# barlettacarmen/CrCNN

Hardware: AMD Instinct MI355X
Metric: encrypted images/sec (higher is better)
Workload: dtype u64

## Files before the change

crcnn_amd/binding.py:

```python
import ctypes
import os
import re

import numpy as np

_HERE = os.path.dirname(os.path.abspath(__file__))
LIB_PATH = os.path.join(_HERE, "lib", "libcrcnn_hip.so")
HEADER = os.path.join(os.path.dirname(_HERE), "include", "crcnn_hip.h")

u64 = ctypes.c_uint64
PU = ctypes.POINTER(u64)
VP = ctypes.c_void_p
CI = ctypes.c_int
SZ = ctypes.c_size_t

COEFF, NTT, NTTP, NTTL, NTTL1, NTTLC, NTTLS = 0, 1, 2, 3, 4, 5, 6


class CrcError(RuntimeError):
    def __init__(self, status, what=""):
        self.status = status
        super().__init__(f"{what}: {_strerror(status)} (status {status}, hip error {_lib.crc_last_hip_error() if _lib else '?'})")


# ... 47 lines not shown
    L.crc_event_create.argtypes = [VP, ctypes.POINTER(VP)]; L.crc_event_destroy.argtypes = [VP, VP]; L.crc_event_record.argtypes = [VP, VP, VP]
    L.crc_event_elapsed_ms.argtypes = [VP, VP, VP, ctypes.POINTER(ctypes.c_float)]
    L.crc_stream_create.argtypes = [VP, ctypes.POINTER(VP)]; L.crc_stream_destroy.argtypes = [VP, VP]; L.crc_stream_wait_event.argtypes = [VP, VP, VP]
    L.crc_host_alloc.argtypes = [VP, SZ, ctypes.POINTER(VP)]; L.crc_host_free.argtypes = [VP, VP]
    L.crc_host_thread_limit.argtypes = []
    L.crc_encode_f32.argtypes = [VP, ctypes.POINTER(ctypes.c_float), SZ, PU, ctypes.POINTER(ctypes.c_int32)]
    L.crc_encode_f64.argtypes = [VP, ctypes.POINTER(ctypes.c_double), SZ, PU, ctypes.POINTER(ctypes.c_int32)]
    L.crc_decode.restype = ctypes.c_double; L.crc_decode.argtypes = [VP, PU]
    L.crc_bn_invstd_f32.argtypes = [ctypes.POINTER(ctypes.c_float), SZ, ctypes.POINTER(ctypes.c_float)]
    L.crc_plain_to_ntt.argtypes = [VP, VP, SZ, VP, VP]
    L.crc_encode_f32_compact.argtypes = [VP, ctypes.POINTER(ctypes.c_float), SZ, PU, ctypes.POINTER(ctypes.c_int32)]
    L.crc_plain_expand.argtypes = [VP, VP, SZ, VP, VP]
    L.crc_plain_to_delta.argtypes = [VP, VP, SZ, CI, VP, VP]
    L.crc_ntt_fwd.argtypes = [VP, VP, SZ, CI, VP]
    L.crc_ntt_inv.argtypes = [VP, VP, SZ, CI, VP]
    L.crc_ntt_fwd_bsk.argtypes = [VP, VP, SZ, VP]
    L.crc_ntt_inv_bsk.argtypes = [VP, VP, SZ, VP]
    L.crc_add.argtypes = [VP, VP, VP, SZ, CI, VP]
    L.crc_add_plain.argtypes = [VP, VP, VP, SZ, SZ, CI, VP]
    L.crc_multiply_plain_ntt.argtypes = [VP, VP, VP, SZ, SZ, CI, VP]
    L.crc_multiply_plain.argtypes = [VP, VP, VP, SZ, SZ, VP]
    L.crc_conv2d_work_bytes.restype = SZ; L.crc_conv2d_work_bytes.argtypes = [VP] + [CI] * 10
    L.crc_conv2d.argtypes = [VP, VP, VP, VP] + [CI] * 11 + [VP, VP, VP]
    L.crc_conv2d_fold_pool.argtypes = [VP, VP, VP, VP] + [CI] * 8 + [VP, VP, VP]
    L.crc_conv2d_hoist_pool.argtypes = [VP, VP, VP, VP] + [CI] * 6 + [VP, VP, VP]
    L.crc_dense_work_bytes.restype = SZ; L.crc_dense_work_bytes.argtypes = [VP, CI, CI, CI, CI]
    L.crc_dense.argtypes = [VP, VP, VP, VP, CI, CI, CI, CI, CI, VP, VP, VP]
    L.crc_pool.argtypes = [VP, VP] + [CI] * 8 + [VP, CI, VP, VP]
    L.crc_batchnorm.argtypes = [VP, VP, CI, CI, CI, CI, VP, VP, CI, VP]
    L.crc_pad.argtypes = [VP, VP] + [CI] * 9 + [VP, VP]
# ... 601 lines not shown
        if isinstance(x, DBuf):
            return x.ptr
        if hasattr(x, "data_ptr"):
            return x.data_ptr()
        return int(x)

    def plain_to_ntt(self, d_plain, count, d_out):
        _chk(self.L.crc_plain_to_ntt(self.c, self.p(d_plain), count, self.p(d_out), self.stream), "crc_plain_to_ntt")

    def plain_to_delta(self, d_plain, count, form, d_out):
        _chk(self.L.crc_plain_to_delta(self.c, self.p(d_plain), count, form, self.p(d_out), self.stream), "crc_plain_to_delta")

    def ntt_fwd(self, d_ct, count, size=2):
        _chk(self.L.crc_ntt_fwd(self.c, self.p(d_ct), count, size, self.stream), "crc_ntt_fwd")

    def ntt_inv(self, d_ct, count, size=2):
        _chk(self.L.crc_ntt_inv(self.c, self.p(d_ct), count, size, self.stream), "crc_ntt_inv")

    def add(self, d_acc, d_b, count, size=2):
        _chk(self.L.crc_add(self.c, self.p(d_acc), self.p(d_b), count, size, self.stream), "crc_add")

    def add_plain(self, d_ct, d_delta, count, group, sign=1):
        _chk(self.L.crc_add_plain(self.c, self.p(d_ct), self.p(d_delta), count, group, sign, self.stream), "crc_add_plain")

    def multiply_plain_ntt(self, d_ct, d_w, count, group, size=2):
        _chk(self.L.crc_multiply_plain_ntt(self.c, self.p(d_ct), self.p(d_w), count, group, size, self.stream), "crc_multiply_plain_ntt")

    def multiply_plain(self, d_ct, d_w, count, group):
        _chk(self.L.crc_multiply_plain(self.c, self.p(d_ct), self.p(d_w), count, group, self.stream), "crc_multiply_plain")

# ... 539 lines not shown
```

crcnn_amd/csrc/abi.hip:

```cpp
#include <cstdlib>
#include <cstring>
#include <vector>
#include "kernels.h"
#include "chacha.h"
#include "work_arena.h"

#define CHECK_CTX(c) do { if (!(c) || (c)->device < 0) return CRC_ERR_INVALID_ARGUMENT; \
        int dev_ = -1; if (hipGetDevice(&dev_) != hipSuccess || dev_ != (c)->device) HIPCHK(hipSetDevice((c)->device)); } while (0)
#define RUN(x) do { int rc_ = (x); if (rc_) return rc_; } while (0)
static inline hipStream_t S(void *s) { return (hipStream_t)s; }
static inline bool form_ok(int f) { return f == CRC_COEFF || f == CRC_NTT; }
static inline bool nform_ok(int f) { return f == CRC_COEFF || f == CRC_NTT || f == CRC_NTTP; }
static inline bool lform_ok(int f) { return nform_ok(f) || f == CRC_NTTL; }
static inline bool limb_in(int f) { return f == CRC_NTTL || f == CRC_NTTLS; }
static inline u64 *work_base(void *d_work) { return WorkArena(d_work).take<u64>(0); }
static inline size_t work_bytes(size_t words) { WorkArena a; a.take<u64>(words); return a.bytes(); }

extern "C" int crc_plain_to_ntt(crc_ctx *c, const uint64_t *d_plain, size_t count, uint64_t *d_out, void *stream)
{
    CHECK_CTX(c); if (!d_plain || !d_out) return CRC_ERR_INVALID_ARGUMENT;
    return k_plain_ntt(c, d_plain, count, 1, true, d_out, S(stream));
}
extern "C" int crc_plain_expand(crc_ctx *c, const uint64_t *d_compact, size_t count, uint64_t *d_plain, void *stream)
{
    CHECK_CTX(c); if (!d_compact || !d_plain) return CRC_ERR_INVALID_ARGUMENT;
    return k_plain_expand(c, d_compact, count, d_plain, S(stream));
}
extern "C" int crc_plain_to_delta(crc_ctx *c, const uint64_t *d_plain, size_t count, int form, uint64_t *d_out, void *stream)
{
    CHECK_CTX(c); if (!d_plain || !d_out || !form_ok(form)) return CRC_ERR_INVALID_ARGUMENT;
    return k_plain_ntt(c, d_plain, count, 2, form == CRC_NTT, d_out, S(stream));
}

extern "C" int crc_ntt_fwd(crc_ctx *c, uint64_t *d_ct, size_t count, int size, void *stream)
{
    CHECK_CTX(c); if (!d_ct || size < 1) return CRC_ERR_INVALID_ARGUMENT;
    return k_ntt_ct(c, false, d_ct, d_ct, count, size, false, S(stream), nullptr, 0, 0);
}
extern "C" int crc_ntt_inv(crc_ctx *c, uint64_t *d_ct, size_t count, int size, void *stream)
{
    CHECK_CTX(c); if (!d_ct || size < 1) return CRC_ERR_INVALID_ARGUMENT;
    return k_ntt_ct(c, true, d_ct, d_ct, count, size, false, S(stream), nullptr, 0, 0);
}
extern "C" int crc_ntt_fwd_bsk(crc_ctx *c, uint64_t *d_rows, size_t count, void *stream)
{
    CHECK_CTX(c); if (!d_rows) return CRC_ERR_INVALID_ARGUMENT;
    return k_ntt_ct(c, false, d_rows, d_rows, count, 1, true, S(stream), nullptr, 0, 0);
}
extern "C" int crc_ntt_inv_bsk(crc_ctx *c, uint64_t *d_rows, size_t count, void *stream)
{
    CHECK_CTX(c); if (!d_rows) return CRC_ERR_INVALID_ARGUMENT;
    return k_ntt_ct(c, true, d_rows, d_rows, count, 1, true, S(stream), nullptr, 0, 0);
}
// ... 105 lines not shown
    L.out_form = out_form == CRC_NTTLC && P == 1 ? CRC_NTTL : out_form;
    L.Bs = conv1_sub_batch(c, B, w, nf, L.out_form);
    L.Xr = a.take<signed char>(k_limb_conv1_image_bytes(c, L.Bs, w, nf));
    if (L.out_form != CRC_NTTLC) L.Ys = a.take<u64>(k_limb_result_words(c, L.Bs, nf, P));
    if (in_form == CRC_COEFF) L.buf = a.take<u64>((size_t)L.Bs * in.xd * in.yd * crc_ct_words(c, 2));
    return L;
}
static int conv2d_limb1(crc_ctx *c, const uint64_t *d_x, const void *d_wl, const uint64_t *d_bias, int B, const Window &in, int nf, int in_form, int out_form,
                        uint64_t *d_y, void *d_work, hipStream_t st, int bxf = 1, int byf = 1)
{
    const int P = in.boxed(bxf, byf).P(), in_cts = in.xd * in.yd;
    WorkArena a(d_work);
    const Limb1Work L = limb1_layout(c, B, in, bxf, byf, nf, in_form, out_form, a);
    out_form = L.out_form;
    const size_t ctw = crc_ct_words(c, 2);
    for (int b0 = 0; b0 < B; b0 += L.Bs) {
        const int Bn = B - b0 < L.Bs ? B - b0 : L.Bs;
        const u64 *xn = d_x + (size_t)b0 * in_cts * ctw; bool packed = in_form == CRC_NTTP;
        if (in_form == CRC_COEFF) { RUN(k_ntt_ct(c, false, xn, L.buf, (size_t)Bn * in_cts, 2, false, st, nullptr, 0, 0, 0, 0)); xn = L.buf; packed = false; }
        RUN(k_limb_conv1(c, xn, packed, L.Xr, (const signed char *)d_wl, L.Ys, out_form == CRC_NTTLC ? (signed char *)d_y : nullptr, B, b0,
            out_form != CRC_COEFF ? d_bias : nullptr, Bn, in, nf, st, bxf, byf));
        if (out_form == CRC_NTTLC) continue;
        if (out_form == CRC_NTTL) return k_limb_result_to_limb(c, L.Ys, (signed char *)d_y, B, nf * P, st);
        RUN(k_limb_result_to_rows(c, L.Ys, d_y + (size_t)b0 * nf * P * ctw, (size_t)Bn * nf * P * 2, out_form == CRC_NTTP, st));
    }
    if (out_form == CRC_COEFF) RUN(k_ntt_ct(c, true, d_y, d_y, (size_t)B * nf * P, 2, false, st, d_bias, 1, (size_t)P, nf));
    return CRC_OK;
}
struct LimbWork { u64 *Ys; signed char *Xl; u64 *buf; };
static LimbWork limb_layout(const crc_ctx *c, int B, const LayerShape &s, int in_form, WorkArena &a)
{
    LimbWork L{};
    L.Ys = a.take<u64>(k_limb_result_words(c, B, s.nf, s.w.P()));
    if (!limb_in(in_form)) L.Xl = a.take<signed char>(k_limb_tensor_bytes(c, B, s.zd, s.w.xd * s.w.yd));
    if (in_form == CRC_COEFF) L.buf = a.take<u64>((size_t)B * s.zd * s.w.xd * s.w.yd * crc_ct_words(c, 2));
    return L;
// ... 1427 lines not shown
```

crcnn_amd/csrc/ctx.cpp:

```cpp
#include "ctx.h"
#include "host_parallel.h"
#include <algorithm>
#include <cstring>
#include <cstdlib>
#include <string>

typedef unsigned __int128 u128;

static thread_local int g_last_hip = 0;
int crc_set_hip_error(hipError_t e) { g_last_hip = (int)e; return CRC_ERR_HIP; }

extern "C" int crc_last_hip_error(void) { return g_last_hip; }
extern "C" int crc_version(void) { return 100; }
extern "C" const char *crc_strerror(int s)
{
    switch (s) {
    case CRC_OK: return "ok";
    case CRC_ERR_INVALID_ARGUMENT: return "invalid argument";
    case CRC_ERR_PARAMETERS: return "encryption parameters are not set correctly";
    case CRC_ERR_HIP: return "HIP runtime error";
    case CRC_ERR_UNSUPPORTED: return "unsupported parameter combination";
    case CRC_ERR_IO: return "I/O error";
    case CRC_ERR_NOT_FOUND: return "not found";
    case CRC_ERR_COMM: return "RCCL error";
// ... 131 lines not shown
    auto geti = [](const char *name, long long dflt) { const char *e = getenv(name); return e && *e ? atoll(e) : dflt; };
    t.no_fold = getenv("CRC_NO_FOLD") ? 1 : 0;
    t.ntt_inv61_loose = getenv("CRC_NTT_INV61_LOOSE") ? 1 : 0;
    t.mfma_order = (int)geti("CRC_MFMA_ORDER", -1);
    t.mfma_variant = (int)geti("CRC_MFMA_VARIANT", 2);
    { const int v = (int)geti("CRC_MFMA_RING", 0); t.mfma_ring = v >= 3 && v <= 5 ? v : 0; }
    { const int v = (int)geti("CRC_CONV1_WAVES", 0); t.conv1_waves = v == 8 || v == 12 ? v : 0; }
    t.conv1_narrow = (int)geti("CRC_CONV1_NARROW", 1);
    { const int v = (int)geti("CRC_CONV1_FORM", 0); t.conv1_form = v == 1 || v == 2 ? v : 0; }
    t.hoist_pool = geti("CRC_HOIST_POOL", 1) ? 1 : 0;
    { const int v = (int)geti("CRC_HOIST_RT", 0); t.hoist_rt = v == 1 || v == 2 ? v : 0; }
    { const int v = (int)geti("CRC_BSGS_JT", 0); t.bsgs_jt = v == 1 || v == 2 ? v : 0; }
    { const int v = (int)geti("CRC_PLANES_BATCH", 0); t.planes_batch = v == 1 || v == 2 ? v : 0; }
    { const int v = (int)geti("CRC_CONV_JT", 0); t.conv_jt = v == 2 || v == 4 || v == 8 ? v : 0; }
    t.conv1_box = geti("CRC_CONV1_BOX", 1) ? 1 : 0;
    { const long long v = geti("CRC_CONV1_PASS_BYTES", 0); t.conv1_pass_bytes = v > 0 ? v : 0; }
    { const int v = (int)geti("CRC_LIMB_PACK_GROUP", 1); t.limb_pack_group = v > 0 ? v : 1; }
    t.mac2_cfg = (int)geti("CRC_MAC2_CFG", 0);
    t.mac_order = (int)geti("CRC_MAC_ORDER", -1);
    t.mac_regstage = (int)geti("CRC_MAC_REGSTAGE", 0);
    t.mac_stream = (int)geti("CRC_MAC_STREAM", 1);
    t.mac2_dbg = (int)geti("CRC_MAC2_DBG", 0);
    t.relin_path = (int)geti("CRC_RELIN_PATH", 0);
    t.sq_path = (int)geti("CRC_SQ_PATH", 0);
    t.sq_chunk = (int)geti("CRC_SQ_CHUNK", 0);
    t.sq_fuse = (int)geti("CRC_SQ_FUSE", -1);
    t.f64_radix = (int)geti("CRC_F64_RADIX", 0);
    t.f64_wave = (int)geti("CRC_F64_WAVE", -1);
    t.ntt_wave = (int)geti("CRC_NTT_WAVE", -1);
    t.mfma_min_steps = (int)geti("CRC_MFMA_MIN_STEPS", 0);
// ... 7 lines not shown
    if (!c || !name) return CRC_ERR_INVALID_ARGUMENT;
    const std::string s(name);
    CrcTuning &t = c->tune;
    if (s == "mfma_order") t.mfma_order = (int)value;
    else if (s == "mfma_variant") t.mfma_variant = (int)value;
    else if (s == "mfma_ring") t.mfma_ring = value >= 3 && value <= 5 ? (int)value : 0;
    else if (s == "conv1_waves") t.conv1_waves = value == 8 || value == 12 ? (int)value : 0;
    else if (s == "conv1_narrow") t.conv1_narrow = (int)value;
    else if (s == "conv1_form") t.conv1_form = value == 1 || value == 2 ? (int)value : 0;
    else if (s == "hoist_pool") t.hoist_pool = value ? 1 : 0;
    else if (s == "hoist_rt") t.hoist_rt = value == 1 || value == 2 ? (int)value : 0;
    else if (s == "bsgs_jt") t.bsgs_jt = value == 1 || value == 2 ? (int)value : 0;
    else if (s == "planes_batch") t.planes_batch = value == 1 || value == 2 ? (int)value : 0;
    else if (s == "conv_jt") t.conv_jt = value == 2 || value == 4 || value == 8 ? (int)value : 0;
    else if (s == "conv1_box") t.conv1_box = value ? 1 : 0;
    else if (s == "conv1_pass_bytes") t.conv1_pass_bytes = value > 0 ? value : 0;
    else if (s == "limb_pack_group") t.limb_pack_group = value > 0 ? (int)value : 1;
    else if (s == "mac2_cfg") t.mac2_cfg = (int)value;
    else if (s == "mac_order") t.mac_order = (int)value;
    else if (s == "mac_regstage") t.mac_regstage = (int)value;
    else if (s == "mac_stream") t.mac_stream = (int)value;
    else if (s == "ntt_inv61_loose") t.ntt_inv61_loose = value ? 1 : 0;
    else if (s == "relin_path") t.relin_path = (int)value;
    else if (s == "sq_path") t.sq_path = (int)value;
    else if (s == "sq_chunk") t.sq_chunk = (int)value;
    else if (s == "sq_fuse") t.sq_fuse = (int)value;
    else if (s == "f64_radix") t.f64_radix = (int)value;
    else if (s == "f64_wave") t.f64_wave = (int)value;
    else if (s == "ntt_wave") t.ntt_wave = (int)value;
    else if (s == "mfma_min_steps") t.mfma_min_steps = (int)value;
// ... 435 lines not shown
```

crcnn_amd/csrc/ctx.h:

```cpp
#pragma once
#include <hip/hip_runtime.h>
#include <atomic>
#include <mutex>
#include <unordered_map>
#include <vector>
#include "modarith.h"
#include "f64mod.h"
#include "../../include/crcnn_hip.h"

#define CRC_MAXK 8
#define CRC_MAXB (CRC_MAXK + 2)

struct PlainParams {
    u64 threshold;
    u64 inc[CRC_MAXK];
    int fast;
    u64 delta[CRC_MAXK];
    u64 uhi[CRC_MAXK];
};

struct BehzParams {
    int k, ka, kb;
    u64 t;
    u64 m_tilde, m_sk;
// ... 49 lines not shown
    ModParams m;
    u64 root, inv_n;
    std::vector<u64> rp, srp, irp2, sirp2;
    std::vector<u64> irp, sirp;
};

struct CrcTuning {
    int no_fold = 0;
    int ntt_inv61_loose = 0;
    int mfma_order = -1;
    int mfma_variant = 2;
    int mfma_ring = 0;
    int conv1_waves = 0;
    int conv1_narrow = 1;
    int conv1_box = 1;
    int hoist_rt = 0;
    int bsgs_jt = 0;
    int planes_batch = 0;
    int conv_jt = 0;
    int hoist_pool = 1;
    int conv1_form = 0;
    long long conv1_pass_bytes = 0;
    int limb_pack_group = 1;
    int mac2_cfg = 0;
    int mac_order = -1;
    int mac_regstage = 0;
    int mac_stream = 1;
    int mac2_dbg = 0;
    int ntt_split = 1;
    int relin_mac_ct = 0;
// ... 67 lines not shown
```

crcnn_amd/csrc/kernels.h:

```cpp
#pragma once
#include "ctx.h"
#include "window.h"

static inline unsigned xcd_grid(size_t groups, unsigned G) { return (unsigned)((groups + 7) / 8 * 8 * G); }

int k_ntt_ct(crc_ctx *c, bool inv, const u64 *src, u64 *dst, size_t count, int size, bool bsk, hipStream_t st,
             const u64 *addend, int add_sign, size_t add_group, int add_mod = 0, int pack_out = 0);
int k_ntt_ct_fwd_mul(crc_ctx *c, u64 *ct, size_t count, const u64 *w, size_t group, hipStream_t st);
int k_ntt_ct_fwd_fma(crc_ctx *c, u64 *ct, size_t count, const u64 *u, const u64 *key, hipStream_t st);
int k_ntt_ct_fwd_negmul(crc_ctx *c, u64 *ct, size_t count, const u64 *sk, hipStream_t st);
int k_ntt_ct_poly0(crc_ctx *c, const u64 *src, u64 *dst, size_t count, hipStream_t st);
int k_ntt_ct_addct(crc_ctx *c, const u64 *src, u64 *dst, size_t count, const u64 *addct, int add_size, hipStream_t st);
int k_ntt_ct_head_add(crc_ctx *c, const u64 *src, int src_size, u64 *dst, size_t count, const u64 *addrows, hipStream_t st);
int k_spread_ntt(crc_ctx *c, const u64 *src, size_t items, u64 *dst, hipStream_t st);
int k_digit_ntt(crc_ctx *c, const u64 *src, int src_size, int src_poly, size_t count, int D, const unsigned char *dig_i, const unsigned char *dig_shift, int dbc,
                u64 *dst, hipStream_t st, int pack_out = 0);
int k_square_intt(crc_ctx *c, const u64 *src, u64 *dst, size_t count, bool bsk, hipStream_t st, const u64 *opt_mul = nullptr, bool *applied = nullptr);
int k_multiply_intt(crc_ctx *c, const u64 *x, const u64 *y, u64 *dst, size_t count, bool bsk, hipStream_t st, const u64 *opt_mul = nullptr, bool *applied = nullptr);
int k_ntt_ct_inv_scaled(crc_ctx *c, const u64 *src, u64 *dst, size_t count, int size, const u64 *mul, const u64 *mul_s, hipStream_t st);
int k_plain_ntt(crc_ctx *c, const u64 *d_plain, size_t count, int mode, bool do_ntt, u64 *d_out, hipStream_t st);
int k_plain_expand(crc_ctx *c, const u64 *d_compact, size_t count, u64 *d_plain, hipStream_t st);
int k_rowwise(crc_ctx *c, u64 *acc, const u64 *b, size_t count, int size, int op, int sign, size_t group, size_t gmod, hipStream_t st);
int k_pool(crc_ctx *c, const u64 *x, u64 *y, int B, int zd, const Window &w, const u64 *mul, hipStream_t st, int pack_out = 0);
int k_pad(crc_ctx *c, const u64 *x, u64 *y, int B, int zd, int xd, int yd, int px0, int px1, int py0, int py1, hipStream_t st);
// ... 103 lines not shown
```

crcnn_amd/csrc/kernels.hip:

```cpp
#include "kernels.h"
#include <type_traits>
#include <cstdlib>

struct NttArgs {
    const u64 *src; u64 *dst;
    const ModParams *mods; const ulonglong2 *w;
    int n, logn;
    int mod_base, mod_count;
    int src_rows_per_item;
    size_t rows;
    int pack_out;
    int src_ct_rows, dst_ct_rows;
    int prologue;
    int D, src_size, src_poly; unsigned long long dig_mask;
    size_t pairs;
    u64 post_mul[CRC_MAXK], post_mul_s[CRC_MAXK];
    const u64 *fma_u, *fma_k;
    unsigned long long fma_group;
    int opt_mul;
    unsigned char dig_i[48], dig_shift[48];
    const u64 *addend; int add_sign; int rows_per_ct; long long add_group;
    int add_mod;
    int add_mode, add_size;
    int fma_neg;
    PlainParams pp;
};

__device__ __forceinline__ u64 plain_lift(u64 c, const PlainParams &pp, int i, const ModParams &m)
{
    if (pp.fast) return c >= pp.threshold ? c + pp.inc[i] : c;
    const u64 r = barrett128(c, 0, m);
    return c >= pp.threshold ? addmod(r, pp.inc[i], m.q) : r;
}

#include "ntt_device.h"
#include "ntt_f64.h"
__device__ __forceinline__ u64 split28v(u64 v) { return (v & 0x0fffffffULL) | ((v >> 28) << 32); }

template <bool INV, bool LAZY, int PRO>
__device__ __forceinline__ void ntt_rows_body(const NttArgs &a)
{
    extern __shared__ u64 sm[];
    const int n = a.n, logn = a.logn, tid = threadIdx.x, nt = blockDim.x;
    size_t row = blockIdx.x;
    if (INV && (PRO == 4 || PRO == 6)) {
        size_t pair; unsigned p;
        if (!xcd_group(blockIdx.x, 3, a.pairs, pair, p)) return;
        row = ((pair / a.mod_count) * 3 + p) * a.mod_count + pair % a.mod_count;
    }
    const int mloc = (int)(row % a.mod_count);
    const int mi = a.mod_base + mloc;
// ... 83 lines not shown
        for (int s = 2 * tid; s < n; s += 2 * nt) {
            ulonglong2 v = sm_load_pair64(sm, s);
            v.x = fin(v.x); v.y = fin(v.y);
            if (add) {
                const ulonglong2 ad = ld2(add + s);
                if (a.add_sign > 0) { v.x = addmod(v.x, ad.x, q); v.y = addmod(v.y, ad.y, q); } else { v.x = submod(v.x, ad.x, q); v.y = submod(v.y, ad.y, q); }
            }
            st2(dst + s, v.x, v.y);
        }
    }
}

template <bool INV, bool LAZY, int PRO>
__global__ void __launch_bounds__(1024) ntt_rows_kernel(NttArgs a) { ntt_rows_body<INV, LAZY, PRO>(a); }

template <bool INV, int PRO, int CS, bool UNS, int FMA = 0>
__global__ void __launch_bounds__(CS == 1 ? 128 : CS == 2 ? 256 : CS == 3 ? 512 : 1024, 4) ntt_rows_wave_kernel(NttArgs a)
{
    constexpr int E = 16 >> CS, C = 1 << CS;
    extern __shared__ u64 sm[];
    const int n = a.n, tid = threadIdx.x;
    size_t row = blockIdx.x;
    if (INV && (PRO == 4 || PRO == 6)) {
        size_t pair; unsigned p;
        if (!xcd_group(blockIdx.x, 3, a.pairs, pair, p)) return;
        row = ((pair / a.mod_count) * 3 + p) * a.mod_count + pair % a.mod_count;
    }
    const int mloc = (int)(row % a.mod_count), mi = a.mod_base + mloc;
    const ModParams m = a.mods[mi];
    const u64 q = m.q, q2 = m.two_q;
    const float rq = 1.0f / (float)((u32)(q >> 32) + 1);
    const ulonglong2 *W = a.w + (size_t)mi * n, *W1 = W + (n >> 1);
    u64 *dst = a.dst + row * (size_t)n;
    auto pt = [&](int c, int e) { return E * tid + e + 1024 * c; };
    if (!INV) {
        const size_t srow = a.dst_ct_rows ? (row / a.dst_ct_rows) * a.src_ct_rows + row % a.dst_ct_rows : (a.src_rows_per_item ? (row / a.mod_count) : row);
        const u64 *src = a.src + srow * (size_t)n;
        u64 x[16];
#pragma unroll
        for (int c = 0; c < C; c++) {
            if constexpr (E == 1) x[c] = src[pt(c, 0)];
            else {
#pragma unroll
                for (int e = 0; e < E; e += 2) { const ulonglong2 v = ld2(src + pt(c, e)); x[c * E + e] = v.x; x[c * E + e + 1] = v.y; }
            }
        }
#pragma unroll
        for (int e = 0; e < E; e++) {
            u64 y[C];
#pragma unroll
            for (int c = 0; c < C; c++) y[c] = x[c * E + e];
            fwd_stages<CS, true>(y, W, 1, 0, q, q2);
#pragma unroll
            for (int c = 0; c < C; c++) sm[swz<3>(pt(c, e))] = y[c];
        }
        __syncthreads();
        const bool fma_lazy = m.fold != 0 && m.bits >= 53;
        u64_local_passes_fwd<true>(sm, W, n, q, q2);
#pragma unroll 2
        for (int u = 0; u < 8; u++) {
// ... 311 lines not shown
                if (a.add_mode == 2) add = a.addend + ((ct * a.add_size + p) * a.mod_count + mloc) * (size_t)n;
                else if (p == 0) { size_t g = ct / a.add_group; if (a.add_mod) g %= a.add_mod; add = a.addend + (g * a.mod_count + mloc) * (size_t)n; }
            }
        } else if (a.addend) add = a.addend + row * (size_t)n;
        for (int s = tid; s < n; s += nt) {
            u64 v = sm[lpad(s)];
            if (LAZY) v = reduce_small(v, q, q2, rq);
            else { v = v >= q2 ? v - q2 : v; v = v >= q ? v - q : v; }
            if (add) v = (INV && a.add_sign < 0) ? submod(v, add[s], q) : addmod(v, add[s], q);
            dst[s] = (!INV && a.pack_out) ? split28v(v) : v;
        }
        __syncthreads();
    }
}

static int ntt_launch(crc_ctx *c, bool inv, NttArgs &a, size_t rows, hipStream_t st)
{
    if (rows == 0) return CRC_OK;
    a.mods = c->d_mods; a.n = c->n; a.logn = c->logn;
    a.w = reinterpret_cast<const ulonglong2 *>(inv ? c->d_irp2 : c->d_rp);
    int nt = c->n / 8; if (nt < 64) nt = 64; if (nt > 1024) nt = 1024;
    size_t lds = (size_t)c->n * 8;
    if (lds > 128 * 1024) return CRC_ERR_UNSUPPORTED;
    bool lazy = true;
    for (int i = a.mod_base; i < a.mod_base + a.mod_count; i++) if (c->tabs[i].m.bits > 57 || c->tabs[i].m.bits < 45) lazy = false;
    const int cus = c->cus;
    if ((a.prologue == 3 && inv) || ((a.prologue == 4 || a.prologue == 5 || a.prologue == 6) && !inv)) return CRC_ERR_INVALID_ARGUMENT;
    const bool two_src = a.prologue == 6;
    if (a.prologue == 4 || two_src) rows = xcd_grid(a.pairs, 3);
    {
        const int sel = c->tune.ntt_wave < 0 ? 47 : c->tune.ntt_wave;
        const int bit = c->n == 8192 ? 0 : c->n == 4096 ? 1 : c->n == 16384 ? (a.prologue ? 3 : 2) : c->n == 2048 ? 5 : -1;
        if (bit >= 0 && ((sel >> bit) & 1) && lazy && !a.addend && (a.prologue == 0 || a.prologue == 4 || a.prologue == 5 || two_src)) {
            lds = (size_t)c->n * 8;
            bool uns = inv && !(sel & 16);
            for (int i = 0; i < a.mod_count; i++) uns = uns && c->tabs[a.mod_base + i].m.q < (1ull << 55);
            if (uns) {
                a.w = reinterpret_cast<const ulonglong2 *>(c->d_irp);
                for (int i = 0; i < a.mod_count; i++) {
                    const HostNtt &T = c->tabs[a.mod_base + i]; const u64 q = T.m.q;
                    const u64 pm = a.prologue == 5 || a.opt_mul ? (u64)(((unsigned __int128)a.post_mul[i] * T.inv_n) % q) : T.inv_n;
                    a.post_mul[i] = pm; a.post_mul_s[i] = (u64)(((unsigned __int128)pm << 64) / q);
                }
                if (a.opt_mul) a.opt_mul = 2;
            }
            const int cs = c->logn - 10;
#define WAVEK(CSV, U) (two_src ? ntt_rows_wave_kernel<true, 6, CSV, U> : a.prologue == 4 ? ntt_rows_wave_kernel<true, 4, CSV, U> : a.prologue == 5 ? ntt_rows_wave_kernel<true, 5, CSV, U> \
                       : inv ? ntt_rows_wave_kernel<true, 0, CSV, U> : ntt_rows_wave_kernel<false, 0, CSV, false>)
// ... 49 lines not shown
    hipLaunchKernelGGL(kern, dim3((unsigned)rows), dim3(nt), lds, st, a);
    HIPCHK(hipGetLastError());
    return CRC_OK;
}

int k_ntt_ct(crc_ctx *c, bool inv, const u64 *src, u64 *dst, size_t count, int size, bool bsk, hipStream_t st,
             const u64 *addend, int add_sign, size_t add_group, int add_mod, int pack_out)
{
    NttArgs a{};
    a.pack_out = inv ? 0 : pack_out;
    a.src = src; a.dst = dst;
    a.mod_base = bsk ? c->k : 0; a.mod_count = bsk ? c->kb : c->k;
    a.addend = addend; a.add_sign = add_sign; a.rows_per_ct = size * a.mod_count; a.add_group = (long long)(add_group ? add_group : 1);
    a.add_mode = 1; a.add_mod = add_mod;
    return ntt_launch(c, inv, a, count * size * a.mod_count, st);
}

int k_ntt_ct_fwd_fma(crc_ctx *c, u64 *ct, size_t count, const u64 *u, const u64 *key, hipStream_t st)
{
    NttArgs a{};
    a.src = ct; a.dst = ct; a.mod_base = 0; a.mod_count = c->k; a.rows_per_ct = 2 * c->k; a.add_group = 1; a.add_mode = 1;
    a.fma_u = u; a.fma_k = key;
    return ntt_launch(c, false, a, count * 2 * c->k, st);
}

int k_ntt_ct_fwd_negmul(crc_ctx *c, u64 *ct, size_t count, const u64 *sk, hipStream_t st)
{
    NttArgs a{};
    a.src = ct; a.dst = ct; a.mod_base = 0; a.mod_count = c->k; a.rows_per_ct = 2 * c->k; a.add_group = 1; a.add_mode = 1;
    a.src_ct_rows = 2 * c->k; a.dst_ct_rows = c->k;
// ... 1003 lines not shown
```

include/crcnn_hip.h:

```cpp
#ifndef CRCNN_HIP_H
#define CRCNN_HIP_H
#include <stddef.h>
#include <stdint.h>

#ifdef __cplusplus
extern "C" {
#endif

typedef struct crc_ctx crc_ctx;

typedef enum {
    CRC_OK = 0,
    CRC_ERR_INVALID_ARGUMENT = -1,
    CRC_ERR_PARAMETERS = -2,
    CRC_ERR_HIP = -3,
    CRC_ERR_UNSUPPORTED = -4,
    CRC_ERR_IO = -5,
    CRC_ERR_NOT_FOUND = -6,
    CRC_ERR_COMM = -7
} crc_status;

enum { CRC_COEFF = 0, CRC_NTT = 1,
       CRC_NTTP = 2,
       CRC_NTTL = 3,
// ... 39 lines not shown
int    crc_encode_f32(const crc_ctx *ctx, const float *h_values, size_t count, uint64_t *h_plain , int32_t *h_coeff_count);
int    crc_encode_f64(const crc_ctx *ctx, const double *h_values, size_t count, uint64_t *h_plain, int32_t *h_coeff_count);
double crc_decode(const crc_ctx *ctx, const uint64_t *h_plain );
#define CRC_PLAIN_COMPACT_LOW   64
#define CRC_PLAIN_COMPACT_HIGH  32
#define CRC_PLAIN_COMPACT_WORDS 96
int    crc_encode_f32_compact(const crc_ctx *ctx, const float *h_values, size_t count, uint64_t *h_compact , int32_t *h_coeff_count);
int    crc_bn_invstd_f32(const float *h_var, size_t count, float *h_invstd);

int crc_plain_to_ntt(crc_ctx *ctx, const uint64_t *d_plain, size_t count, uint64_t *d_out, void *stream);
int crc_plain_expand(crc_ctx *ctx, const uint64_t *d_compact , size_t count, uint64_t *d_plain , void *stream);
int crc_plain_to_delta(crc_ctx *ctx, const uint64_t *d_plain, size_t count, int form, uint64_t *d_out, void *stream);

int crc_ntt_fwd(crc_ctx *ctx, uint64_t *d_ct, size_t count, int size, void *stream);
int crc_ntt_inv(crc_ctx *ctx, uint64_t *d_ct, size_t count, int size, void *stream);
int crc_ntt_fwd_bsk(crc_ctx *ctx, uint64_t *d_rows, size_t count, void *stream);
int crc_ntt_inv_bsk(crc_ctx *ctx, uint64_t *d_rows, size_t count, void *stream);

int crc_add(crc_ctx *ctx, uint64_t *d_acc, const uint64_t *d_b, size_t count, int size, void *stream);
int crc_add_plain(crc_ctx *ctx, uint64_t *d_ct, const uint64_t *d_delta, size_t count, size_t group, int sign, void *stream);
int crc_multiply_plain_ntt(crc_ctx *ctx, uint64_t *d_ct, const uint64_t *d_w_ntt, size_t count, size_t group, int size, void *stream);
int crc_multiply_plain(crc_ctx *ctx, uint64_t *d_ct, const uint64_t *d_w_ntt, size_t count, size_t group, void *stream);

size_t crc_conv2d_work_bytes(const crc_ctx *ctx, int B, int zd, int xd, int yd, int xs, int ys, int xf, int yf, int nf, int in_form);
int crc_conv2d(crc_ctx *ctx, const uint64_t *d_x, const uint64_t *d_w_ntt, const uint64_t *d_bias_delta,
               int B, int zd, int xd, int yd, int xs, int ys, int xf, int yf, int nf,
               int in_form, int out_form, uint64_t *d_y, void *d_work, void *stream);
int crc_conv2d_fold_pool(crc_ctx *ctx, const uint64_t *d_w_ntt, const uint64_t *d_bias_delta_ntt, const uint64_t *d_div_ntt, int nf, int zd, int xf, int yf,
                         int cxs, int cys, int pxf, int pyf, uint64_t *d_w_out, uint64_t *d_bias_out, void *stream);
int crc_conv2d_hoist_pool(crc_ctx *ctx, const uint64_t *d_w_ntt, const uint64_t *d_bias_delta_ntt, const uint64_t *d_div_ntt, int nf, int zd, int xf, int yf,
// ... 253 lines not shown
```

Before: 831.4.

## Sum pooled-box input pixels in coefficient form before forward NTT in conv1

Adds a box-summing forward NTT kernel that adds the bxf×byf input ciphertext rows (a box filter folded into the first limb convolution) in coefficient form, then transforms only the summed rows. Linearity of the NTT lets conv1 run with a 1×1 box on the smaller summed window instead of transforming every input pixel and summing afterwards. This cuts the number of NTTs and the convolution's box loop. The cost is more strided source loads per row and a new XCD-aware block ordering. It is enabled by default through a tune knob.

```diff
diff --git a/crcnn_amd/binding.py b/crcnn_amd/binding.py
--- a/crcnn_amd/binding.py
+++ b/crcnn_amd/binding.py
@@ -85,6 +85,7 @@
     L.crc_plain_to_delta.argtypes = [VP, VP, SZ, CI, VP, VP]
     L.crc_ntt_fwd.argtypes = [VP, VP, SZ, CI, VP]
     L.crc_ntt_inv.argtypes = [VP, VP, SZ, CI, VP]
+    L.crc_ntt_fwd_box.argtypes = [VP, VP, VP] + [CI] * 7 + [VP]
     L.crc_ntt_fwd_bsk.argtypes = [VP, VP, SZ, VP]
     L.crc_ntt_inv_bsk.argtypes = [VP, VP, SZ, VP]
     L.crc_add.argtypes = [VP, VP, VP, SZ, CI, VP]
@@ -716,6 +717,9 @@
     def ntt_fwd(self, d_ct, count, size=2):
         _chk(self.L.crc_ntt_fwd(self.c, self.p(d_ct), count, size, self.stream), "crc_ntt_fwd")
 
+    def ntt_fwd_box(self, d_src, d_dst, B, xd, yd, bxf, byf, xs, ys):
+        _chk(self.L.crc_ntt_fwd_box(self.c, self.p(d_src), self.p(d_dst), B, xd, yd, bxf, byf, xs, ys, self.stream), "crc_ntt_fwd_box")
+
     def ntt_inv(self, d_ct, count, size=2):
         _chk(self.L.crc_ntt_inv(self.c, self.p(d_ct), count, size, self.stream), "crc_ntt_inv")
 
diff --git a/crcnn_amd/csrc/abi.hip b/crcnn_amd/csrc/abi.hip
--- a/crcnn_amd/csrc/abi.hip
+++ b/crcnn_amd/csrc/abi.hip
@@ -37,6 +37,11 @@
     CHECK_CTX(c); if (!d_ct || size < 1) return CRC_ERR_INVALID_ARGUMENT;
     return k_ntt_ct(c, false, d_ct, d_ct, count, size, false, S(stream), nullptr, 0, 0);
 }
+extern "C" int crc_ntt_fwd_box(crc_ctx *c, const uint64_t *d_src, uint64_t *d_dst, int B, int xd, int yd, int bxf, int byf, int xs, int ys, void *stream)
+{
+    CHECK_CTX(c); if (!d_src || !d_dst) return CRC_ERR_INVALID_ARGUMENT;
+    return k_ntt_ct_box(c, d_src, d_dst, B, xd, yd, bxf, byf, xs, ys, S(stream));
+}
 extern "C" int crc_ntt_inv(crc_ctx *c, uint64_t *d_ct, size_t count, int size, void *stream)
 {
     CHECK_CTX(c); if (!d_ct || size < 1) return CRC_ERR_INVALID_ARGUMENT;
@@ -172,12 +177,16 @@
     const Limb1Work L = limb1_layout(c, B, in, bxf, byf, nf, in_form, out_form, a);
     out_form = L.out_form;
     const size_t ctw = crc_ct_words(c, 2);
+    const bool sum_first = in_form == CRC_COEFF && bxf * byf > 1 && c->tune.box_ntt != 0 && k_ntt_ct_box_supported(c, bxf, byf);
+    const Window wsum = in.boxed(bxf, byf);
     for (int b0 = 0; b0 < B; b0 += L.Bs) {
         const int Bn = B - b0 < L.Bs ? B - b0 : L.Bs;
         const u64 *xn = d_x + (size_t)b0 * in_cts * ctw; bool packed = in_form == CRC_NTTP;
-        if (in_form == CRC_COEFF) { RUN(k_ntt_ct(c, false, xn, L.buf, (size_t)Bn * in_cts, 2, false, st, nullptr, 0, 0, 0, 0)); xn = L.buf; packed = false; }
+        if (sum_first) RUN(k_ntt_ct_box(c, xn, L.buf, Bn, in.xd, in.yd, bxf, byf, in.xs, in.ys, st));
+        else if (in_form == CRC_COEFF) RUN(k_ntt_ct(c, false, xn, L.buf, (size_t)Bn * in_cts, 2, false, st, nullptr, 0, 0, 0, 0));
+        if (in_form == CRC_COEFF) { xn = L.buf; packed = false; }
         RUN(k_limb_conv1(c, xn, packed, L.Xr, (const signed char *)d_wl, L.Ys, out_form == CRC_NTTLC ? (signed char *)d_y : nullptr, B, b0,
-            out_form != CRC_COEFF ? d_bias : nullptr, Bn, in, nf, st, bxf, byf));
+            out_form != CRC_COEFF ? d_bias : nullptr, Bn, sum_first ? wsum : in, nf, st, sum_first ? 1 : bxf, sum_first ? 1 : byf));
         if (out_form == CRC_NTTLC) continue;
         if (out_form == CRC_NTTL) return k_limb_result_to_limb(c, L.Ys, (signed char *)d_y, B, nf * P, st);
         RUN(k_limb_result_to_rows(c, L.Ys, d_y + (size_t)b0 * nf * P * ctw, (size_t)Bn * nf * P * 2, out_form == CRC_NTTP, st));
diff --git a/crcnn_amd/csrc/ctx.cpp b/crcnn_amd/csrc/ctx.cpp
--- a/crcnn_amd/csrc/ctx.cpp
+++ b/crcnn_amd/csrc/ctx.cpp
@@ -169,6 +169,7 @@
     { const int v = (int)geti("CRC_PLANES_BATCH", 0); t.planes_batch = v == 1 || v == 2 ? v : 0; }
     { const int v = (int)geti("CRC_CONV_JT", 0); t.conv_jt = v == 2 || v == 4 || v == 8 ? v : 0; }
     t.conv1_box = geti("CRC_CONV1_BOX", 1) ? 1 : 0;
+    { const int v = (int)geti("CRC_BOX_NTT", 1); t.box_ntt = v >= 0 && v <= 2 ? v : 1; }
     { const long long v = geti("CRC_CONV1_PASS_BYTES", 0); t.conv1_pass_bytes = v > 0 ? v : 0; }
     { const int v = (int)geti("CRC_LIMB_PACK_GROUP", 1); t.limb_pack_group = v > 0 ? v : 1; }
     t.mac2_cfg = (int)geti("CRC_MAC2_CFG", 0);
@@ -206,6 +207,7 @@
     else if (s == "planes_batch") t.planes_batch = value == 1 || value == 2 ? (int)value : 0;
     else if (s == "conv_jt") t.conv_jt = value == 2 || value == 4 || value == 8 ? (int)value : 0;
     else if (s == "conv1_box") t.conv1_box = value ? 1 : 0;
+    else if (s == "box_ntt") t.box_ntt = value >= 0 && value <= 2 ? (int)value : 1;
     else if (s == "conv1_pass_bytes") t.conv1_pass_bytes = value > 0 ? value : 0;
     else if (s == "limb_pack_group") t.limb_pack_group = value > 0 ? (int)value : 1;
     else if (s == "mac2_cfg") t.mac2_cfg = (int)value;
diff --git a/crcnn_amd/csrc/ctx.h b/crcnn_amd/csrc/ctx.h
--- a/crcnn_amd/csrc/ctx.h
+++ b/crcnn_amd/csrc/ctx.h
@@ -87,6 +87,7 @@
     int conv1_waves = 0;
     int conv1_narrow = 1;
     int conv1_box = 1;
+    int box_ntt = 1;
     int hoist_rt = 0;
     int bsgs_jt = 0;
     int planes_batch = 0;
diff --git a/crcnn_amd/csrc/kernels.h b/crcnn_amd/csrc/kernels.h
--- a/crcnn_amd/csrc/kernels.h
+++ b/crcnn_amd/csrc/kernels.h
@@ -6,6 +6,8 @@
 
 int k_ntt_ct(crc_ctx *c, bool inv, const u64 *src, u64 *dst, size_t count, int size, bool bsk, hipStream_t st,
              const u64 *addend, int add_sign, size_t add_group, int add_mod = 0, int pack_out = 0);
+bool k_ntt_ct_box_supported(const crc_ctx *c, int bxf, int byf);
+int k_ntt_ct_box(crc_ctx *c, const u64 *src, u64 *dst, int B, int xd, int yd, int bxf, int byf, int xs, int ys, hipStream_t st);
 int k_ntt_ct_fwd_mul(crc_ctx *c, u64 *ct, size_t count, const u64 *w, size_t group, hipStream_t st);
 int k_ntt_ct_fwd_fma(crc_ctx *c, u64 *ct, size_t count, const u64 *u, const u64 *key, hipStream_t st);
 int k_ntt_ct_fwd_negmul(crc_ctx *c, u64 *ct, size_t count, const u64 *sk, hipStream_t st);
diff --git a/crcnn_amd/csrc/kernels.hip b/crcnn_amd/csrc/kernels.hip
--- a/crcnn_amd/csrc/kernels.hip
+++ b/crcnn_amd/csrc/kernels.hip
@@ -1,4 +1,5 @@
 #include "kernels.h"
+#include "nttbox.h"
 #include <type_traits>
 #include <cstdlib>
 
@@ -24,6 +25,7 @@
     int add_mode, add_size;
     int fma_neg;
     PlainParams pp;
+    NttBox box; int box_order; unsigned box_images;
 };
 
 __device__ __forceinline__ u64 plain_lift(u64 c, const PlainParams &pp, int i, const ModParams &m)
@@ -35,6 +37,7 @@
 
 #include "ntt_device.h"
 #include "ntt_f64.h"
+#include "limbred.h"
 __device__ __forceinline__ u64 split28v(u64 v) { return (v & 0x0fffffffULL) | ((v >> 28) << 32); }
 
 template <bool INV, bool LAZY, int PRO>
@@ -148,10 +151,11 @@
 template <bool INV, bool LAZY, int PRO>
 __global__ void __launch_bounds__(1024) ntt_rows_kernel(NttArgs a) { ntt_rows_body<INV, LAZY, PRO>(a); }
 
-template <bool INV, int PRO, int CS, bool UNS, int FMA = 0>
-__global__ void __launch_bounds__(CS == 1 ? 128 : CS == 2 ? 256 : CS == 3 ? 512 : 1024, 4) ntt_rows_wave_kernel(NttArgs a)
+template <bool INV, int PRO, int CS, bool UNS, int FMA = 0, bool BOX = false>
+__global__ void __launch_bounds__(CS == 1 ? 128 : CS == 2 ? 256 : CS == 3 ? 512 : 1024, BOX && CS <= 2 ? 5 : 4) ntt_rows_wave_kernel(NttArgs a)
 {
     constexpr int E = 16 >> CS, C = 1 << CS;
+    static_assert(!BOX || (!INV && PRO == 0 && FMA == 0), "the box belongs to the plain forward transform");
     extern __shared__ u64 sm[];
     const int n = a.n, tid = threadIdx.x;
     size_t row = blockIdx.x;
@@ -160,7 +164,12 @@
         if (!xcd_group(blockIdx.x, 3, a.pairs, pair, p)) return;
         row = ((pair / a.mod_count) * 3 + p) * a.mod_count + pair % a.mod_count;
     }
-    const int mloc = (int)(row % a.mod_count), mi = a.mod_base + mloc;
+    NttBoxRow br{};
+    if constexpr (BOX) {
+        if (!nttbox_block_row(a.box_order, blockIdx.x, a.box_images, a.box, a.mod_count, br)) return;
+        row = nttbox_row_of(br, a.box, a.mod_count);
+    }
+    const int mloc = BOX ? br.mod : (int)(row % a.mod_count), mi = a.mod_base + mloc;
     const ModParams m = a.mods[mi];
     const u64 q = m.q, q2 = m.two_q;
     const float rq = 1.0f / (float)((u32)(q >> 32) + 1);
@@ -171,6 +180,33 @@
         const size_t srow = a.dst_ct_rows ? (row / a.dst_ct_rows) * a.src_ct_rows + row % a.dst_ct_rows : (a.src_rows_per_item ? (row / a.mod_count) : row);
         const u64 *src = a.src + srow * (size_t)n;
         u64 x[16];
+        if constexpr (BOX) {
+            const int terms = a.box.bxf * a.box.byf;
+            auto load8 = [&](u64 (&v)[8], int h, int t) {
+                const int ta = t / a.box.byf, tb = t - ta * a.box.byf;
+                const u64 *tp = a.src + nttbox_src_row(br, a.box, a.mod_count, ta, tb) * (size_t)n;
+#pragma unroll
+                for (int i = 0; i < 8; i += (E == 1 ? 1 : 2)) {
+                    const int p = h * 8 + i, c = p / E, e = p % E;
+                    if constexpr (E == 1) v[i] = tp[pt(c, 0)];
+                    else { const ulonglong2 w = ld2(tp + pt(c, e)); v[i] = w.x; v[i + 1] = w.y; }
+                }
+            };
+#pragma unroll
+            for (int h = 0; h < 2; h++) {
+                u64 cur[8], nxt[8], acc[8];
+#pragma unroll
+                for (int i = 0; i < 8; i++) acc[i] = 0;
+                load8(cur, h, 0);
+                for (int t = 1; t < terms; t++) {
+                    load8(nxt, h, t);
+#pragma unroll
+                    for (int i = 0; i < 8; i++) { acc[i] += cur[i]; cur[i] = nxt[i]; }
+                }
+#pragma unroll
+                for (int i = 0; i < 8; i++) x[h * 8 + i] = sum_reduce16(acc[i] + cur[i], q);
+            }
+        } else {
 #pragma unroll
         for (int c = 0; c < C; c++) {
             if constexpr (E == 1) x[c] = src[pt(c, 0)];
@@ -178,6 +214,7 @@
 #pragma unroll
                 for (int e = 0; e < E; e += 2) { const ulonglong2 v = ld2(src + pt(c, e)); x[c * E + e] = v.x; x[c * E + e + 1] = v.y; }
             }
+        }
         }
 #pragma unroll
         for (int e = 0; e < E; e++) {
@@ -519,6 +556,17 @@
     }
 }
 
+static bool ntt_lazy_moduli(const crc_ctx *c, int mod_base, int mod_count)
+{
+    for (int i = mod_base; i < mod_base + mod_count; i++) if (c->tabs[i].m.bits > 57 || c->tabs[i].m.bits < 45) return false;
+    return true;
+}
+static bool ntt_wave_ring(const crc_ctx *c, bool with_prologue)
+{
+    const int sel = c->tune.ntt_wave < 0 ? 47 : c->tune.ntt_wave;
+    const int bit = c->n == 8192 ? 0 : c->n == 4096 ? 1 : c->n == 16384 ? (with_prologue ? 3 : 2) : c->n == 2048 ? 5 : -1;
+    return bit >= 0 && ((sel >> bit) & 1);
+}
 static int ntt_launch(crc_ctx *c, bool inv, NttArgs &a, size_t rows, hipStream_t st)
 {
     if (rows == 0) return CRC_OK;
@@ -527,16 +575,14 @@
     int nt = c->n / 8; if (nt < 64) nt = 64; if (nt > 1024) nt = 1024;
     size_t lds = (size_t)c->n * 8;
     if (lds > 128 * 1024) return CRC_ERR_UNSUPPORTED;
-    bool lazy = true;
-    for (int i = a.mod_base; i < a.mod_base + a.mod_count; i++) if (c->tabs[i].m.bits > 57 || c->tabs[i].m.bits < 45) lazy = false;
+    const bool lazy = ntt_lazy_moduli(c, a.mod_base, a.mod_count);
     const int cus = c->cus;
     if ((a.prologue == 3 && inv) || ((a.prologue == 4 || a.prologue == 5 || a.prologue == 6) && !inv)) return CRC_ERR_INVALID_ARGUMENT;
     const bool two_src = a.prologue == 6;
     if (a.prologue == 4 || two_src) rows = xcd_grid(a.pairs, 3);
     {
         const int sel = c->tune.ntt_wave < 0 ? 47 : c->tune.ntt_wave;
-        const int bit = c->n == 8192 ? 0 : c->n == 4096 ? 1 : c->n == 16384 ? (a.prologue ? 3 : 2) : c->n == 2048 ? 5 : -1;
-        if (bit >= 0 && ((sel >> bit) & 1) && lazy && !a.addend && (a.prologue == 0 || a.prologue == 4 || a.prologue == 5 || two_src)) {
+        if (ntt_wave_ring(c, a.prologue != 0) && lazy && !a.addend && (a.prologue == 0 || a.prologue == 4 || a.prologue == 5 || two_src)) {
             lds = (size_t)c->n * 8;
             bool uns = inv && !(sel & 16);
             for (int i = 0; i < a.mod_count; i++) uns = uns && c->tabs[a.mod_base + i].m.q < (1ull << 55);
@@ -616,6 +662,33 @@
     a.addend = addend; a.add_sign = add_sign; a.rows_per_ct = size * a.mod_count; a.add_group = (long long)(add_group ? add_group : 1);
     a.add_mode = 1; a.add_mod = add_mod;
     return ntt_launch(c, inv, a, count * size * a.mod_count, st);
+}
+
+#define NTT_BOX_ORDER 1
+bool k_ntt_ct_box_supported(const crc_ctx *c, int bxf, int byf)
+{
+    return bxf >= 1 && byf >= 1 && bxf * byf <= NTTBOX_MAX_TERMS && ntt_wave_ring(c, false) && ntt_lazy_moduli(c, 0, c->k);
+}
+int k_ntt_ct_box(crc_ctx *c, const u64 *src, u64 *dst, int B, int xd, int yd, int bxf, int byf, int xs, int ys, hipStream_t st)
+{
+    const NttBox g = nttbox_make(xd, yd, bxf, byf, xs, ys);
+    if (B < 0 || !nttbox_ok(g) || src == dst) return CRC_ERR_INVALID_ARGUMENT;
+    if (!k_ntt_ct_box_supported(c, bxf, byf)) return CRC_ERR_UNSUPPORTED;
+    if (B == 0) return CRC_OK;
+    NttArgs a{};
+    a.src = src; a.dst = dst; a.mods = c->d_mods; a.n = c->n; a.logn = c->logn; a.w = reinterpret_cast<const ulonglong2 *>(c->d_rp);
+    a.mod_base = 0; a.mod_count = c->k;
+    a.box = g; a.box_images = (unsigned)B; a.box_order = c->tune.box_ntt == 2 ? 1 - NTT_BOX_ORDER : NTT_BOX_ORDER;
+    const size_t grid = nttbox_grid(a.box_order, (size_t)B, g, c->k);
+    if (grid > 0x7fffffffULL) return CRC_ERR_INVALID_ARGUMENT;
+    const int cs = c->logn - 10;
+    auto kw = cs == 1 ? ntt_rows_wave_kernel<false, 0, 1, false, 0, true> : cs == 2 ? ntt_rows_wave_kernel<false, 0, 2, false, 0, true>
+            : cs == 3 ? ntt_rows_wave_kernel<false, 0, 3, false, 0, true> : ntt_rows_wave_kernel<false, 0, 4, false, 0, true>;
+    const size_t lds = (size_t)c->n * 8;
+    { const int rc = crc_ctx_ensure_lds(c, (const void *)kw, lds); if (rc) return rc; }
+    hipLaunchKernelGGL(kw, dim3((unsigned)grid), dim3(c->n / 16), lds, st, a);
+    HIPCHK(hipGetLastError());
+    return CRC_OK;
 }
 
 int k_ntt_ct_fwd_fma(crc_ctx *c, u64 *ct, size_t count, const u64 *u, const u64 *key, hipStream_t st)
diff --git a/crcnn_amd/csrc/nttbox.h b/crcnn_amd/csrc/nttbox.h
--- /dev/null
+++ b/crcnn_amd/csrc/nttbox.h
@@ -0,0 +1,47 @@
+#pragma once
+#include <stddef.h>
+#include "modarith.h"
+
+struct NttBox { int xd, yd, xdo, ydo, bxf, byf, xs, ys; };
+CRC_HD NttBox nttbox_make(int xd, int yd, int bxf, int byf, int xs, int ys) { return {xd, yd, xd - (bxf - 1) * xs, yd - (byf - 1) * ys, bxf, byf, xs, ys}; }
+CRC_HD bool nttbox_ok(const NttBox &g) { return g.xd >= 1 && g.yd >= 1 && g.bxf >= 1 && g.byf >= 1 && g.xs >= 1 && g.ys >= 1 && g.xdo >= 1 && g.ydo >= 1; }
+#define NTTBOX_MAX_TERMS 9
+
+CRC_HD size_t nttbox_pixels(const NttBox &g) { return (size_t)g.xdo * g.ydo; }
+CRC_HD size_t nttbox_planes(size_t B, int k) { return B * 2 * (size_t)k; }
+CRC_HD size_t nttbox_rows(size_t B, const NttBox &g, int k) { return nttbox_planes(B, k) * nttbox_pixels(g); }
+
+struct NttBoxRow { u32 b; int r, c, poly, mod; };
+CRC_HD size_t nttbox_row_of(const NttBoxRow &o, const NttBox &g, int k)
+{
+    return ((((size_t)o.b * g.xdo + (size_t)o.r) * g.ydo + (size_t)o.c) * 2 + (size_t)o.poly) * (size_t)k + (size_t)o.mod;
+}
+CRC_HD size_t nttbox_src_row(const NttBoxRow &o, const NttBox &g, int k, int a, int bb)
+{
+    return ((((size_t)o.b * g.xd + (size_t)(o.r + a * g.xs)) * g.yd + (size_t)(o.c + bb * g.ys)) * 2 + (size_t)o.poly) * (size_t)k + (size_t)o.mod;
+}
+
+CRC_HD size_t nttbox_grid(int order, size_t B, const NttBox &g, int k)
+{
+    if (order == 0) return nttbox_rows(B, g, k);
+    return (nttbox_planes(B, k) + 7) / 8 * 8 * nttbox_pixels(g);
+}
+CRC_HD bool nttbox_block_row(int order, u32 blk, u32 B, const NttBox &g, int k, NttBoxRow &o)
+{
+    const u32 P = (u32)g.xdo * (u32)g.ydo, planes = B * 2 * (u32)k;
+    u32 px, plane;
+    if (order == 0) {
+        const u32 pk = 2 * (u32)k, bp = blk / pk, pm = blk - bp * pk;
+        o.b = bp / P; px = bp - o.b * P;
+        plane = o.b * pk + pm;
+    } else {
+        const u32 xcd = blk & 7, slot = blk >> 3, sp = slot / P;
+        px = slot - sp * P; plane = sp * 8 + xcd;
+        o.b = plane / (2 * (u32)k);
+    }
+    if (plane >= planes) return false;
+    const u32 pm = plane - o.b * 2 * (u32)k;
+    o.poly = pm >= (u32)k ? 1 : 0; o.mod = (int)(pm - (o.poly ? (u32)k : 0));
+    o.r = (int)(px / (u32)g.ydo); o.c = (int)(px - (u32)o.r * (u32)g.ydo);
+    return true;
+}
diff --git a/include/crcnn_hip.h b/include/crcnn_hip.h
--- a/include/crcnn_hip.h
+++ b/include/crcnn_hip.h
@@ -77,6 +77,7 @@
 
 int crc_ntt_fwd(crc_ctx *ctx, uint64_t *d_ct, size_t count, int size, void *stream);
 int crc_ntt_inv(crc_ctx *ctx, uint64_t *d_ct, size_t count, int size, void *stream);
+int crc_ntt_fwd_box(crc_ctx *ctx, const uint64_t *d_src, uint64_t *d_dst, int B, int xd, int yd, int bxf, int byf, int xs, int ys, void *stream);
 int crc_ntt_fwd_bsk(crc_ctx *ctx, uint64_t *d_rows, size_t count, void *stream);
 int crc_ntt_inv_bsk(crc_ctx *ctx, uint64_t *d_rows, size_t count, void *stream);
 
```

Measured after the change: 846.1 (median of 6 runs). +1.8%, better.
